# ntampellini/FIRECODE

Measured on AMD Instinct MI355X. Metric: conformer-pair RMSD alignments/s, higher is better.
Workload: dtype f64

## Files before the change

firecode_amd/csrc/fc_api_prune.cpp:

```cpp
#include <algorithm>
#include <chrono>
#include <cmath>
#include <cstdlib>
#include <functional>
#include <memory>

#include "fc_internal.h"
#include "fc_kabsch_math.h"

namespace fc {

struct LadderKs {
  int n;
  int64_t k[24];
};
__global__ void k_store_ladder_ks(LadderKs a, int64_t *__restrict__ out) {
  if ((int)threadIdx.x < a.n) out[threadIdx.x] = a.k[threadIdx.x];
}

static int make_selection(const uint8_t *atom_mask, int64_t A_all, std::vector<int32_t> &sel) {
  sel.clear();
  for (int64_t a = 0; a < A_all; ++a)
    if (atom_mask == nullptr || atom_mask[a]) sel.push_back((int32_t)a);
  if (sel.empty()) return set_error(FC_E_INVALID, "atom_mask selects no atom");
// ... 307 lines not shown
    FC_TRY(sync());
  }
  unpack_ladder_result(e, words, cnt_host, job.mask_out, job.levels, job.survivors, job.counters_out);
  return FC_OK;
}

static void note_candidates(fc_ensemble *e, unsigned long long refined, unsigned long long similar) {
  int guard = 0;
  for (fc_ensemble *w = e->head ? e->head : e; w != nullptr && guard < 8; w = w->twin, ++guard) {
    w->last_candidates = (int64_t)refined;
    w->last_similar = (int64_t)similar;
  }
  Context &c = ctx();
  c.hint_A = e->A, c.hint_N = e->N, c.hint_candidates = (int64_t)refined, c.hint_similar = (int64_t)similar;
}

static bool ladder_collect(fc_ensemble *e, int64_t slot, uint8_t *mask_out, int64_t *levels,
                           int64_t *survivors, unsigned long long *counters_out, int64_t slot_stride = 0) {
  const uint64_t *words = slot_words(slot, e->W, slot_stride), *cnt_host = slot_counters(slot, e->W, slot_stride);
  note_candidates(e, cnt_host[6], cnt_host[2]);
  if (cnt_host[9] == 0) return false;
  unpack_ladder_result(e, words, cnt_host, mask_out, levels, survivors, counters_out);
  return true;
}

static int ensemble_twin(fc_ensemble *ens, fc_ensemble **out) {
  if (!ens->twin) {
    std::unique_ptr<fc_ensemble> t(new (std::nothrow) fc_ensemble);
    if (!t) return set_error(FC_E_NOMEM, "host allocation failed");
    t->epoch = ens->epoch;
    t->N = ens->N, t->A = ens->A, t->Npad = ens->Npad, t->W = ens->W;
    t->Xs.alias(ens->Xs), t->Xa.alias(ens->Xa), t->G.alias(ens->G);
    if (ens->xsf_valid) t->Xsf.alias(ens->Xsf), t->sub.alias(ens->sub), t->xsf_valid = true;
    if (ens->xh_valid) t->Xh.alias(ens->Xh), t->xh_valid = true, t->xh_scale = ens->xh_scale;
    t->g_max = ens->g_max;
    t->head = ens->head ? ens->head : ens;
    t->last_candidates = ens->last_candidates, t->last_similar = ens->last_similar;
    FC_TRY(t->counters.reserve(kCounters * sizeof(uint64_t)));
    ens->twin = t.release();
  }
  *out = ens->twin;
  return FC_OK;
}

static int64_t owned_pairs(int64_t N, int64_t row_block, int64_t rank, int64_t world) {
  int64_t n = 0;
  const int64_t nb = ceil_div(N, row_block);
  for (int64_t lb = 0, b; (b = global_block(lb, rank, world)) < nb; ++lb)
    for (int64_t i = b * row_block; i < std::min(N, (b + 1) * row_block); ++i) n += N - 1 - i;
  return n;
}
static int64_t owned_pairs(const fc_ensemble *ens) { return owned_pairs(ens->N, ens->row_block, ens->rank, ens->world); }

static void fill_stats(int64_t *stats, int64_t pairs, const unsigned long long *cnt, int64_t s4, int64_t s5) {
  stats[0] = pairs, stats[1] = (int64_t)cnt[1], stats[2] = (int64_t)cnt[2], stats[3] = (int64_t)cnt[3];
  stats[4] = s4, stats[5] = s5;
}

static int ladder_workspace(fc_ensemble *e, int64_t N, size_t *bits_bytes = nullptr) {
  e->N = N, e->Npad = ceil_div(N, 64) * 64, e->W = e->Npad / 64;
  e->row_block = 64;
  FC_TRY(e->maskA.reserve((size_t)e->Npad));
  FC_TRY(e->maskB.reserve((size_t)e->Npad));
  FC_TRY(e->mbits.reserve((size_t)e->W * sizeof(uint64_t)));
  FC_TRY(e->counters.reserve(kCounters * sizeof(uint64_t)));
  const int64_t rows = ceil_div(N, e->row_block) * e->row_block;
// ... 1836 lines not shown
```

firecode_amd/csrc/fc_common.h:

```cpp
#pragma once

#include <hip/hip_runtime.h>

#include <cstdarg>
#include <cstdint>
#include <cstdio>
#include <cstring>
#include <mutex>
#include <new>
#include <string>
#include <vector>

#include "../../include/fc_hip.h"
#include "fc_items.h"
#include "fc_tuning.h"

namespace fc {

std::string &last_error();
int set_error(int code, const char *fmt, ...);

#define FC_HIP_TRY(expr)                                                              \
  do {                                                                                \
    hipError_t _e = (expr);                                                           \
// ... 215 lines not shown
  int64_t ref_stride = 0;
  const uint64_t *ref_bits = nullptr;
  const int64_t *excl_offsets = nullptr;
  const int64_t *excl_atoms = nullptr;
  int64_t excl_sets = 0;
  int64_t max_newbonds = 0;
  int64_t *counts_out = nullptr;
  uint8_t *ok_out = nullptr;
  const int64_t *offsets = nullptr;
  int64_t *bonds_out = nullptr;
};
int bond_changes(const BondJob &job);

constexpr double kScreenMargin = 1e-6;
constexpr unsigned long long kRefineLanesMin = 1ull << 17;

constexpr size_t kCounters = 64 + 20 * 16;
constexpr int kCntLevel = 64, kCntLevelStride = 16;


}

struct fc_ensemble {
  uint64_t epoch = 0;
  int64_t N = 0, A = 0;
  int64_t Npad = 0, W = 0;
  fc::DevBuf Xs;
  fc::DevBuf Xa;
  fc::DevBuf G;
  fc::DevBuf Xsf;
  fc::DevBuf sub;
  fc::DevBuf unitq;
  bool xsf_valid = false;
  fc::DevBuf Xh;
  bool xh_valid = false;
  double xh_scale = 0.0;
  double g_max = -1.0;
  bool g_max_pending = false;
  std::vector<int32_t> sel_host;
  fc::DevBuf bits;
  fc::DevBuf cand;
  fc::DevBuf pairq;
  int64_t pairq_cap = 0;
  fc::DevBuf simq;
  fc::DevBuf bk, bk_off, bk_list, sortq;
  int64_t bk_buckets = 0;
  int64_t last_candidates = -1;
  int64_t last_similar = -1;
  fc::DevBuf bits_full;
  fc::DevBuf item_table;
  int64_t item_key[4] = {-1, -1, -1, -1}, item_total = 0;
  std::vector<uint64_t> item_host;
  fc::DevBuf gathered;
  fc::DevBuf msg_send, msg_recv;
  fc::DevBuf energies;
  fc::DevBuf maskA, maskB;
  fc::DevBuf mbits;
  fc::DevBuf ladder;
  fc::DevBuf ladder_k;
  fc::DevBuf levelmask;
  std::vector<int64_t> ladder_k_host;
  int ladder_k_n = -1;
  int64_t ladder_k_mpg = -1;
  fc::DevBuf counters;
  int64_t rank = 0, world = 1, row_block = 64;
  int64_t rows_local = 0;
// ... 11 lines not shown
```

firecode_amd/csrc/fc_items.h:

```cpp
#pragma once

#include <algorithm>
#include <cstdint>
#include <utility>
#include <vector>

#if defined(__HIPCC__) || defined(__CUDACC__)
#define FC_ITEMS_HD __host__ __device__
#else
#define FC_ITEMS_HD
#endif

namespace fc {

FC_ITEMS_HD inline int64_t global_block(int64_t local_block, int64_t rank, int64_t world) {
  return local_block * world + ((local_block & 1) ? (world - 1 - rank) : rank);
}
inline int64_t local_block_count(int64_t n_gblocks, int64_t rank, int64_t world) {
  int64_t n = 0;
  while (global_block(n, rank, world) < n_gblocks) ++n;
  return n;
}

constexpr uint64_t kItemFirstHalf = 1ull << 31, kItemSecondHalf = 1ull << 63;
constexpr int kItemChunkShift = 58, kItemChunkMax = 16;
FC_ITEMS_HD inline int64_t item_tile(uint64_t it) { return (int64_t)(it & 0x7fffffffull); }
FC_ITEMS_HD inline int64_t item_block(uint64_t it) { return (int64_t)((it >> 32) & 0x3ffffffull); }
FC_ITEMS_HD inline int item_blocks(uint64_t it) { return (int)((it >> kItemChunkShift) & 15ull) + 1; }

struct ItemPlan {
  int64_t N = 0, rank = 0, world = 1;
  int64_t row_block = 128, tc = 64;
  int64_t NT = 0, n_lblocks = 0;
  bool halves = false;
  int64_t tail = 0;
  bool real_columns_only = false;
  int64_t chunk = 1;
  bool tail_order = true;
};

template <class F>
inline void item_units(uint64_t it, const ItemPlan &p, F visit) {
  const int64_t jt = item_tile(it), lb = item_block(it), j0 = jt * p.tc, tpb = p.row_block / 16;
  int64_t it_first = 0, it_last = tpb * item_blocks(it);
  if (it & kItemFirstHalf) it_last = tpb / 2;
  if (it & kItemSecondHalf) it_first = tpb / 2;
  const int64_t i0 = global_block(lb, p.rank, p.world) * p.row_block;
  if (i0 >= p.N || j0 + p.tc - 1 <= i0) return;
  for (int64_t t = it_first; t < it_last; ++t) {
    const int64_t ib = global_block(lb + t / tpb, p.rank, p.world) * p.row_block + (t % tpb) * 16;
    if (ib >= p.N) break;
    if (j0 + p.tc - 1 <= ib) break;
    for (int64_t cs = 0; cs < p.tc / 16; ++cs) {
      if (j0 + (cs + 1) * 16 - 1 <= ib) continue;
      if (j0 + cs * 16 >= p.N) continue;
      visit(ib, j0 + cs * 16);
    }
  }
}

inline std::vector<uint64_t> build_items(const ItemPlan &p) {
// ... 46 lines not shown
```

firecode_amd/csrc/fc_kabsch.hip:

```cpp
#include <type_traits>

#include "fc_internal.h"
#include <vector>
#include "fc_kabsch_math.h"

#include <algorithm>
#include <cstdlib>

namespace fc {

__global__ void __launch_bounds__(256)
k_prep(const double *__restrict__ coords, int64_t N, int64_t A_all, const int32_t *__restrict__ sel,
       int64_t A, int center, int64_t Npad, double *__restrict__ Xs, double *__restrict__ G,
       double *__restrict__ Xa, unsigned long long *__restrict__ gmax_bits,
       const int32_t *__restrict__ conf_idx) {
  const int64_t n = (int64_t)blockIdx.x * blockDim.x + threadIdx.x;
  if (n >= Npad) return;
  for (int64_t a = A; a < ((A + 3) & ~(int64_t)3); ++a) {
    Xs[(a * 3 + 0) * Npad + n] = 0.0;
    Xs[(a * 3 + 1) * Npad + n] = 0.0;
    Xs[(a * 3 + 2) * Npad + n] = 0.0;
  }
  if (n >= N) {
    for (int64_t a = 0; a < A; ++a) {
// ... 525 lines not shown
        acc[k][0] = fma(x, qx, acc[k][0]);
        acc[k][1] = fma(x, qy, acc[k][1]);
        acc[k][2] = fma(x, qz, acc[k][2]);
        acc[k][3] = fma(y, qx, acc[k][3]);
        acc[k][4] = fma(y, qy, acc[k][4]);
        acc[k][5] = fma(y, qz, acc[k][5]);
        acc[k][6] = fma(z, qx, acc[k][6]);
        acc[k][7] = fma(z, qy, acc[k][7]);
        acc[k][8] = fma(z, qz, acc[k][8]);
      }
    }
#pragma unroll
    for (int k = 0; k < TI; ++k) {
      const int64_t i = ib + k;
      const double Gp = G[i];
      bool may = kabsch_may_be_below<ENANT>(acc[k], Gp + Gq, A_thr2);
      may = may && (j > i) && (j < N) && (i < N);
      const uint64_t word = __ballot(may);
      push_pairs(word, may, (unsigned)i, (unsigned)j, pairq, Q, counters, lane);
      if (lane == 0 && i < N) {
        const int64_t lrow = (int64_t)(lb * IB) + (int64_t)it * TI + k;
        bits[lrow * W + jt] = word;
        if (word) {
          const unsigned long long slot = atomicAdd(&counters[4], 1ull);
          cand[slot] = (uint32_t)(lrow * W + jt);
        }
      }
    }
  }
}

typedef double d4_t __attribute__((ext_vector_type(4)));

template <int NW, int MODE = 0, int TC = 64, bool EIG = false, bool ENANT = false>
__global__ void __launch_bounds__(NW * 64, 2)
k_simbits_screen_mfma(const double *__restrict__ Xs, const double *__restrict__ G, int64_t N,
                      int64_t Npad, int A, double A_thr2, int IB, int64_t rank, int64_t world,
                      uint64_t *__restrict__ bits, int64_t W, uint32_t *__restrict__ cand,
                      unsigned long long *__restrict__ counters, uint64_t *__restrict__ pairq,
                      unsigned long long Q, const uint64_t *__restrict__ item_table, unsigned long long n_items,
                      double *__restrict__ rmsd_out = nullptr, const unsigned long long *__restrict__ gate = nullptr,
                      double *__restrict__ maxdev_out = nullptr) {
  static_assert(!EIG || MODE == 2, "EIG: the complete alignments");
  static_assert(!ENANT || MODE == 0, "ENANT: the screen only");
  constexpr bool VALUES = MODE != 0;
  constexpr int NT = MODE == 2 ? 1 : 2;
  static_assert(TC == 64 || ((TC == 32 || TC == 16) && MODE == 2), "column tiles: 64, or 32 / 16 for the complete alignments");
  constexpr int NU = (TC / 16) / NT;
  constexpr int KPR = TC == 64 ? 2 : 4;
  constexpr int SST = 2048 / TC;
  constexpr int CST = TC == 64 ? 256 : 128;
  auto koff = [](int sl) { return TC == 16 ? (sl >> 1) * 384 + (sl & 1) * 64 : sl * (12 * TC); };
  if (gate != nullptr && *gate == 0ull) return;
  extern __shared__ double lds[];
  const int tid = threadIdx.x;
  const int lane = tid & 63;
  const int wv = __builtin_amdgcn_readfirstlane(tid >> 6);
  const int KS = (A + 3) >> 2;
  double *__restrict__ ldsG = lds + (TC == 16 ? ((KS + 1) >> 1) * 384 : KS * 12 * TC);
  uint64_t *__restrict__ stageQ = reinterpret_cast<uint64_t *>(ldsG + TC + IB);
  uint32_t *__restrict__ stageW = reinterpret_cast<uint32_t *>(stageQ + kStagePairs);
  unsigned *__restrict__ stageN = reinterpret_cast<unsigned *>(stageW + kStageWords);
#ifdef FC_TIMELINE
  unsigned long long *tl = MODE == 2 ? reinterpret_cast<unsigned long long *>(bits) : reinterpret_cast<unsigned long long *>(rmsd_out);
  constexpr bool TL = MODE == 0 || MODE == 2;
#endif
  const unsigned long long b = blockIdx.x;
  if (b >= n_items) return;
#ifdef FC_TIMELINE
  if (TL && tl && tid == 0) {
    tl[(size_t)b * 4] = wall_clock64();
    tl[(size_t)b * 4 + 3] = b;
  }
#endif
  int64_t jt, lb;
  int it_first = 0, it_last = IB >> 4;
// ... 191 lines not shown
          {
            double B4[4][9], GG[4], Q44[4][4], nq4[4], lam4[4];
#pragma unroll
            for (int r = 0; r < 4; ++r) {
              GG[r] = Gp + ldsG[cs * 16 + 4 * kq + r];
#pragma unroll
              for (int e = 0; e < 9; ++e) B4[r][e] = acc[t][e][r];
            }
            kabsch_quaternion_qcp_lean4(B4, GG, Q44, nq4, ok4, EIG ? lam4 : nullptr);
            if constexpr (EIG) {
              const double k_small = 2e-10 / (double)A;
#pragma unroll
              for (int r = 0; r < 4; ++r) {
                msdA4[r] = GG[r] - 2.0 * lam4[r];
                if (!(msdA4[r] > k_small * GG[r] * GG[r])) ok4[r] = false, msdA4[r] = 0.0;
              }
            }
#pragma unroll
            for (int r = 0; r < 4; ++r) {
              if (!ok4[r]) Q44[r][0] = 1.0, Q44[r][1] = 0.0, Q44[r][2] = 0.0, Q44[r][3] = 0.0, nq4[r] = 1.0;
              neg_rotation_from_raw_quaternion(Q44[r], nq4[r], nR[r]);
            }
          }
          typedef double d2_t __attribute__((ext_vector_type(2)));
          const double *__restrict__ qcol = lds + cs * SST + 4 * kq;
          const double *__restrict__ prow_u = Xs + ib;
          const unsigned l15u = (unsigned)l15;
          const int n_rounds = (A + 1) >> 1, n_groups = n_rounds >> 1;
          const bool odd_round = (n_rounds & 1) != 0;
          double ssq[4] = {0.0, 0.0, 0.0, 0.0}, mx[4] = {0.0, 0.0, 0.0, 0.0};
          const int64_t Npad3 = 3 * Npad;
          const double *__restrict__ pa0 = prow_u, *__restrict__ pa1 = prow_u + Npad, *__restrict__ pa2 = prow_u + 2 * Npad;
          const double *__restrict__ qg = qcol;
          auto load_pq = [&](auto u_, double (&P)[3], d2_t (&Qv)[3][2]) {
            constexpr int u = decltype(u_)::value;
            const double *__restrict__ ql = qg + (u / KPR) * 128 + (u % KPR) * 16;
#pragma unroll
            for (int c = 0; c < 3; ++c) {
              Qv[c][0] = *reinterpret_cast<const d2_t *>(ql + c * CST);
              Qv[c][1] = *reinterpret_cast<const d2_t *>(ql + c * CST + 2);
            }
            P[0] = pa0[l15u];
            P[1] = pa1[l15u];
            P[2] = pa2[l15u];
            pa0 += Npad3;
            pa1 += Npad3;
            pa2 += Npad3;
          };
          auto accumulate = [&](const double (&P)[3], const d2_t (&Qv)[3][2]) {
#pragma clang fp contract(fast)
#pragma unroll
            for (int r = 0; r < 4; ++r) {
              const double qx = Qv[0][r >> 1][r & 1], qy = Qv[1][r >> 1][r & 1], qz = Qv[2][r >> 1][r & 1];
              const double dx = fma(nR[r][0], qx, fma(nR[r][1], qy, fma(nR[r][2], qz, P[0])));
              const double dy = fma(nR[r][3], qx, fma(nR[r][4], qy, fma(nR[r][5], qz, P[1])));
              const double dz = fma(nR[r][6], qx, fma(nR[r][7], qy, fma(nR[r][8], qz, P[2])));
              const double s2 = fma(dz, dz, fma(dy, dy, dx * dx));
              if constexpr (!EIG) ssq[r] += s2;
              asm("v_max_f64 %0, %1, %2" : "=v"(mx[r]) : "v"(mx[r]), "v"(s2));
            }
          };
          using U0 = std::integral_constant<int, 0>;
          using U1 = std::integral_constant<int, 1>;
          using U2 = std::integral_constant<int, 2>;
          using U3 = std::integral_constant<int, 3>;
          double PA[3], PB[3];
          d2_t QA[3][2], QB[3][2];
          load_pq(U0{}, PA, QA);
          for (int g = 0; g < n_groups; ++g) {
            load_pq(U1{}, PB, QB);
            __builtin_amdgcn_sched_barrier(0);
            accumulate(PA, QA);
            __builtin_amdgcn_sched_barrier(0);
            load_pq(U2{}, PA, QA);
            __builtin_amdgcn_sched_barrier(0);
            accumulate(PB, QB);
            __builtin_amdgcn_sched_barrier(0);
            load_pq(U3{}, PB, QB);
            __builtin_amdgcn_sched_barrier(0);
            accumulate(PA, QA);
            __builtin_amdgcn_sched_barrier(0);
            qg = TC == 16 ? qcol + koff(g + 1) : qg + 12 * TC;
            if (g + 1 < n_groups || odd_round) load_pq(U0{}, PA, QA);
            __builtin_amdgcn_sched_barrier(0);
            accumulate(PB, QB);
            __builtin_amdgcn_sched_barrier(0);
          }
          if (odd_round) {
            load_pq(U1{}, PB, QB);
            __builtin_amdgcn_sched_barrier(0);
            accumulate(PA, QA);
            __builtin_amdgcn_sched_barrier(0);
            accumulate(PB, QB);
          }
          if constexpr (EIG) {
#pragma unroll
            for (int r = 0; r < 4; ++r) ssq[r] = msdA4[r];
          }
          const bool row_in = i < n32;
          double *__restrict__ ro = rmsd_out + (int64_t)i * N + jb;
          double *__restrict__ mo = maxdev_out + (int64_t)i * N + jb;
          const double invA = 1.0 / (double)A;
          if (row_in && jb > i && jb + 3 < n32 && ((((int64_t)i * N) & 1) == 0)) {
            *reinterpret_cast<d2_t *>(ro) = d2_t{fc_sqrt_nonneg(ssq[0] * invA), fc_sqrt_nonneg(ssq[1] * invA)};
            *reinterpret_cast<d2_t *>(ro + 2) = d2_t{fc_sqrt_nonneg(ssq[2] * invA), fc_sqrt_nonneg(ssq[3] * invA)};
            *reinterpret_cast<d2_t *>(mo) = d2_t{fc_sqrt_nonneg(mx[0]), fc_sqrt_nonneg(mx[1])};
            *reinterpret_cast<d2_t *>(mo + 2) = d2_t{fc_sqrt_nonneg(mx[2]), fc_sqrt_nonneg(mx[3])};
          } else {
#pragma unroll
            for (int r = 0; r < 4; ++r) {
              const int j = jb + r;
              if (row_in && j >= i && j < n32) {
                ro[r] = j == i ? 0.0 : fc_sqrt_nonneg(ssq[r] * invA);
                mo[r] = j == i ? 0.0 : fc_sqrt_nonneg(mx[r]);
              }
            }
          }
#pragma unroll
          for (int r = 0; r < 4; ++r) {
            const int j = jb + r;
            const bool redo = row_in && (j > i) && (j < n32) && !ok4[r];
            stage_pairs(__ballot(redo), redo, (unsigned)i, (unsigned)j, stageQ, stageN, pairq, Q, counters, lane);
          }
          continue;
        }
#pragma unroll
        for (int r = 0; r < 4; ++r) {
// ... 1751 lines not shown

static int screen_item_table(fc_ensemble *e, int64_t NT, int64_t n_lblocks, bool halves = true, int64_t tc = 64, int64_t chunk = 0,
                             bool tail_order = true) {
  const int64_t rb_key = (((e->row_block * 2 + (halves ? 1 : 0)) * 128 + tc) * 32 + chunk) * 2 + (tail_order ? 1 : 0);
  if (e->item_key[0] == e->N && e->item_key[1] == e->rank && e->item_key[2] == e->world &&
      e->item_key[3] == rb_key)
    return FC_OK;
  e->item_total = 0;
  e->item_key[0] = e->N; e->item_key[1] = e->rank; e->item_key[2] = e->world; e->item_key[3] = rb_key;
  ItemPlan plan;
  plan.N = e->N; plan.rank = e->rank; plan.world = e->world;
  plan.row_block = e->row_block; plan.tc = tc; plan.NT = NT; plan.n_lblocks = n_lblocks;
  plan.tail = 2 * (int64_t)ctx().n_cu;
  if (const char *v = getenv("FC_SCREEN_TAIL_SLOTS")) plan.tail = std::max<int64_t>(0, std::strtoll(v, nullptr, 10));
  plan.halves = halves && e->row_block == 128 && e->A <= 52;
  plan.real_columns_only = chunk > 0;
  plan.chunk = std::max<int64_t>(1, chunk);
  plan.tail_order = tail_order;
  std::vector<uint64_t> items = build_items(plan);
  if (items.empty() || items.size() >= (1ull << 31)) return FC_OK;
  FC_TRY(e->item_table.reserve(items.size() * sizeof(uint64_t)));
  e->item_host.swap(items);
  FC_TRY(h2d(e->item_table.p, e->item_host.data(), e->item_host.size() * sizeof(uint64_t)));
  e->item_total = (int64_t)e->item_host.size();
  return FC_OK;
}

int prebuild_screen_items(fc_ensemble *e) {
  const int64_t n_lblocks = local_block_count(ceil_div(e->N, e->row_block), e->rank, e->world);
  if (n_lblocks <= 0 || (e->Npad >> 6) == 0) return FC_OK;
  return screen_item_table(e, e->Npad >> 6, n_lblocks, true, 64);
}

template <int NW, int TC, bool EIG>
static int launch_complete_variant(fc_ensemble *e, dim3 grid, size_t lds_m, double A_small, int64_t rb, int64_t rank, int64_t world,
                                   unsigned long long *cnt, const uint64_t *item_table_dev, unsigned long long n_items,
                                   double *rmsd_dev, double *maxdev_dev, uint64_t *timeline_dev) {
  if (lds_m > 64 * 1024) {
    hipError_t err = hipFuncSetAttribute(reinterpret_cast<const void *>(k_simbits_screen_mfma<NW, 2, TC, EIG>),
                                         hipFuncAttributeMaxDynamicSharedMemorySize, (int)lds_m);
    if (err != hipSuccess) return set_error(FC_E_HIP, "hipFuncSetAttribute failed: %s", hipGetErrorString(err));
  }
  hipLaunchKernelGGL((k_simbits_screen_mfma<NW, 2, TC, EIG>), grid, dim3(NW * 64), lds_m, ctx().stream, e->Xs.as<double>(),
                     e->G.as<double>(), e->N, e->Npad, (int)e->A, A_small, (int)rb, rank, world, timeline_dev, e->W, nullptr, cnt,
                     e->pairq.as<uint64_t>(), (unsigned long long)e->pairq_cap, item_table_dev, n_items, rmsd_dev, nullptr,
                     maxdev_dev);
  return FC_OK;
}

int launch_rmsd_values(fc_ensemble *e, double small_rmsd, double *rmsd_dev, double *maxdev_dev, int64_t rank,
                       int64_t world, bool explicit_sum) {
  const int64_t rb = 128;
  const int64_t n_lblocks = local_block_count(ceil_div(e->N, rb), rank, world);
  if (n_lblocks <= 0) return FC_OK;
  const size_t lds_64 = ((size_t)((e->A + 3) / 4) * 4 * 3 * 64 + 64 + (size_t)rb) * sizeof(double) + kStageBytes;
  const size_t lds_32 = ((size_t)((e->A + 3) / 4) * 4 * 3 * 32 + 32 + (size_t)rb) * sizeof(double) + kStageBytes;
  const size_t lds_16 = ((size_t)(((e->A + 3) / 4 + 1) / 2) * 384 + 16 + (size_t)rb) * sizeof(double) + kStageBytes;
  const bool narrow = lds_64 > kLdsLimit && maxdev_dev != nullptr;
  const int64_t tc = !narrow ? 64 : (lds_32 <= kLdsLimit ? 32 : 16);
  const size_t lds_m = tc == 64 ? lds_64 : (tc == 32 ? lds_32 : lds_16);
  const int64_t NT = e->Npad / tc;
  if (lds_m > kLdsLimit || NT == 0)
    return set_error(FC_E_LIMIT, "A=%lld atoms exceed the LDS column tile of the value kernel", (long long)e->A);
  const bool fits32 = (uint64_t)((e->A + 3) / 4 * 4) * 3 * (uint64_t)e->Npad < (1ull << 32) &&
                      96 * (uint64_t)e->Npad < (1ull << 32);
  if (!fits32) return set_error(FC_E_LIMIT, "ensemble too large for 32-bit operand offsets");
  auto *cnt = reinterpret_cast<unsigned long long *>(e->counters.p);
  const bool two_blocks = 2 * lds_m <= kLdsLimit;
  const bool complete = maxdev_dev != nullptr;
  const void *fn = two_blocks ? reinterpret_cast<const void *>(k_simbits_screen_mfma<4, 1>)
                              : reinterpret_cast<const void *>(k_simbits_screen_mfma<8, 1>);
  if (!complete && lds_m > 64 * 1024) {
    hipError_t err = hipFuncSetAttribute(fn, hipFuncAttributeMaxDynamicSharedMemorySize, (int)lds_m);
    if (err != hipSuccess) return set_error(FC_E_HIP, "hipFuncSetAttribute failed: %s", hipGetErrorString(err));
  }
  const double A_small = (double)e->A * small_rmsd * small_rmsd;
  const int64_t saved_rank = e->rank, saved_world = e->world, saved_rb = e->row_block;
  e->rank = rank; e->world = world; e->row_block = rb;
  int64_t chunk = 0;
  bool tail_order = true;
  if (complete) {
    chunk = two_blocks && !narrow ? kCompleteRowChunk : 1;
    if (const char *v = getenv("FC_COMPLETE_ROW_CHUNK")) chunk = std::min<int64_t>(kItemChunkMax, std::max<int64_t>(1, std::strtoll(v, nullptr, 10)));
    if (const char *v = getenv("FC_COMPLETE_TAIL_ORDER")) tail_order = atoi(v) != 0;
  }
  const int rc_tbl = screen_item_table(e, NT, n_lblocks, true, tc, chunk, tail_order);
  e->rank = saved_rank; e->world = saved_world; e->row_block = saved_rb;
  e->item_key[3] = -1;
  if (rc_tbl != FC_OK) return rc_tbl;
  const int compact = e->item_total > 0 ? 1 : 0;
  const unsigned long long n_items =
      compact ? (unsigned long long)e->item_total : (unsigned long long)NT * (unsigned long long)n_lblocks;
  const uint64_t *item_table_dev = compact ? e->item_table.as<uint64_t>() : nullptr;
  if (n_items >= (1ull << 31)) return set_error(FC_E_LIMIT, "too many value-kernel items for one launch");
  const dim3 grid((unsigned)n_items);
  uint64_t *timeline_dev = nullptr;
#ifdef FC_TIMELINE
  static DevBuf tlbuf;
  const bool timeline = complete && getenv("FC_TIMELINE_OUT") != nullptr;
  if (timeline) {
    FC_TRY(tlbuf.reserve(n_items * 4 * sizeof(uint64_t)));
    FC_HIP_TRY(hipMemsetAsync(tlbuf.p, 0, n_items * 4 * sizeof(uint64_t), ctx().stream));
    timeline_dev = tlbuf.as<uint64_t>();
  }
#endif
#define FC_LAUNCH_VALUES(NW_, MODE_)                                                                      \
  hipLaunchKernelGGL((k_simbits_screen_mfma<NW_, MODE_>), grid, dim3(NW_ * 64), lds_m, ctx().stream,      \
                     e->Xs.as<double>(), e->G.as<double>(), e->N, e->Npad, (int)e->A, A_small, (int)rb,   \
                     rank, world, nullptr, e->W, nullptr, cnt, e->pairq.as<uint64_t>(),                   \
                     (unsigned long long)e->pairq_cap, item_table_dev, n_items, rmsd_dev, nullptr, maxdev_dev)
  const char *eig_env = getenv("FC_COMPLETE_EIG");
  const bool eig = complete && !(eig_env && atoi(eig_env) == 0) && !explicit_sum;
#define FC_LAUNCH_COMPLETE(NW_, TC_)                                                                                        \
  FC_TRY((eig ? launch_complete_variant<NW_, TC_, true>(e, grid, lds_m, A_small, rb, rank, world, cnt, item_table_dev, n_items, \
                                                       rmsd_dev, maxdev_dev, timeline_dev)                                 \
              : launch_complete_variant<NW_, TC_, false>(e, grid, lds_m, A_small, rb, rank, world, cnt, item_table_dev,     \
                                                        n_items, rmsd_dev, maxdev_dev, timeline_dev)))
  if (narrow && tc == 32) {
    FC_LAUNCH_COMPLETE(8, 32);
  } else if (narrow) {
    FC_LAUNCH_COMPLETE(8, 16);
  } else if (complete) {
    if (two_blocks) FC_LAUNCH_COMPLETE(4, 64);
    else FC_LAUNCH_COMPLETE(8, 64);
  } else {
    if (two_blocks) FC_LAUNCH_VALUES(4, 1);
    else FC_LAUNCH_VALUES(8, 1);
  }
#undef FC_LAUNCH_COMPLETE
#undef FC_LAUNCH_VALUES
  FC_TRY(check_launch("k_simbits_screen_mfma<values>"));
#ifdef FC_TIMELINE
  if (timeline) {
    std::vector<uint64_t> h(n_items * 4);
    FC_HIP_TRY(hipMemcpyAsync(h.data(), tlbuf.p, h.size() * sizeof(uint64_t), hipMemcpyDeviceToHost, ctx().stream));
    FC_HIP_TRY(hipStreamSynchronize(ctx().stream));
    if (FILE *f = fopen(getenv("FC_TIMELINE_OUT"), "wb")) {
      const uint64_t head[2] = {(uint64_t)n_items, compact ? 1ull : 0ull};
      fwrite(head, sizeof(uint64_t), 2, f);
      fwrite(h.data(), sizeof(uint64_t), h.size(), f);
      if (compact) fwrite(e->item_host.data(), sizeof(uint64_t), e->item_host.size(), f);
      fclose(f);
    }
  }
#endif
  if (ctx().mark_after_screen) (void)hipEventRecord(ctx().mark_after_screen, ctx().stream);
  hipLaunchKernelGGL(k_rmsd_fix_small, dim3((unsigned)(ctx().n_cu * 4)), dim3(256), 0, ctx().stream,
                     e->Xa.as<double>(), (int)e->A, e->N, e->pairq.as<uint64_t>(), cnt,
                     (unsigned long long)e->pairq_cap, rmsd_dev, maxdev_dev);
  return check_launch("k_rmsd_fix_small");
}

__global__ void __launch_bounds__(256)
k_gather_matrix_pairs(const double *__restrict__ rmsd_m, const double *__restrict__ maxdev_m, int64_t N,
                      const int64_t *__restrict__ pi, const int64_t *__restrict__ pj, int64_t P,
                      double *__restrict__ rmsd_out, double *__restrict__ maxdev_out) {
  const int64_t p = (int64_t)blockIdx.x * blockDim.x + threadIdx.x;
  if (p >= P) return;
  int64_t i = pi[p], j = pj[p];
  if (i > j) { const int64_t t = i; i = j; j = t; }
  rmsd_out[p] = rmsd_m[i * N + j];
  maxdev_out[p] = maxdev_m[i * N + j];
// ... 13 lines not shown
  const int64_t bi = blockIdx.y, bj = blockIdx.x;
  if (bj < bi) return;
  const int tx = threadIdx.x & 31, ty = threadIdx.x >> 5;
  for (int r = ty; r < 32; r += 8) {
    const int64_t i = bi * 32 + r, j = bj * 32 + tx;
    tile[r][tx] = (i < N && j < N) ? m[i * N + j] : 0.0;
  }
  __syncthreads();
  for (int r = ty; r < 32; r += 8) {
    const int64_t j = bj * 32 + r, i = bi * 32 + tx;
    if (i < N && j < N && j > i) m[j * N + i] = tile[tx][r];
  }
}

int launch_mirror_upper(double *m_dev, int64_t N) {
  if (N < 2) return FC_OK;
  const unsigned nb = (unsigned)ceil_div(N, 32);
  hipLaunchKernelGGL(k_mirror_upper, dim3(nb, nb), dim3(256), 0, ctx().stream, m_dev, N);
  return check_launch("k_mirror_upper");
}

int launch_scatter_pairs(const uint64_t *pairs_dev, int64_t n_pairs, int64_t N, int64_t W,
                         uint64_t *bits_dev) {
  if (n_pairs == 0) return FC_OK;
  hipLaunchKernelGGL(k_scatter_pairs, dim3((unsigned)ceil_div(n_pairs, 256)), dim3(256), 0,
                     ctx().stream, pairs_dev, n_pairs, N, W, bits_dev);
  return check_launch("k_scatter_pairs");
}

int launch_prep_begin(fc_ensemble *e) {
  auto *gmax_bits = reinterpret_cast<unsigned long long *>(e->counters.p) + (kCounters - 1);
  FC_HIP_TRY(hipMemsetAsync(gmax_bits, 0, sizeof(unsigned long long), ctx().stream));
  e->xsf_valid = false;
  e->xh_valid = false;
  e->g_max = -1.0;
  return FC_OK;
}
bool prep_by_tiles(int64_t A_all) {
  const size_t lds_tile = (size_t)kPrepTile * (size_t)(A_all * 3 + 1) * sizeof(double) + (size_t)A_all * sizeof(int) + 8;
  return lds_tile + 2048 <= kLdsLimit && (uint64_t)kPrepTile * (uint64_t)(A_all * 3 + 1) < (1ull << 31) &&
         !getenv("FC_PREP_LANES");
}
int launch_prep_tiles(const double *coords_dev, int64_t N, int64_t A_all, const int32_t *sel_dev, int64_t A, int center,
                      fc_ensemble *e, const int32_t *conf_idx_dev, int64_t tile0, int64_t n_tiles) {
  if (n_tiles <= 0) return FC_OK;
  auto *gmax_bits = reinterpret_cast<unsigned long long *>(e->counters.p) + (kCounters - 1);
  constexpr int64_t kPer64 = 64 / kPrepTile;
  const size_t lds_tile = (size_t)kPrepTile * (size_t)(A_all * 3 + 1) * sizeof(double) + (size_t)A_all * sizeof(int) + 8;
  if (lds_tile > 64 * 1024)
    FC_HIP_TRY(hipFuncSetAttribute(reinterpret_cast<const void *>(k_prep_tile<kPrepTile>),
                                   hipFuncAttributeMaxDynamicSharedMemorySize, (int)lds_tile));
  hipLaunchKernelGGL(k_prep_tile<kPrepTile>, dim3((unsigned)(n_tiles * kPer64)), dim3(256), lds_tile, ctx().stream, coords_dev, N,
                     A_all, sel_dev, A, center, e->Npad, e->Xs.as<double>(), e->G.as<double>(), e->Xa.as<double>(), gmax_bits,
                     conf_idx_dev, tile0 * kPer64);
  return check_launch("k_prep_tile");
}
int launch_prep_body(const double *coords_dev, int64_t N, int64_t A_all, const int32_t *sel_dev, int64_t A, int center,
                     fc_ensemble *e, const int32_t *conf_idx_dev);
int launch_prep(const double *coords_dev, int64_t N, int64_t A_all, const int32_t *sel_dev,
                int64_t A, int center, fc_ensemble *e, const int32_t *conf_idx_dev) {
  FC_TRY(launch_prep_begin(e));
  return launch_prep_body(coords_dev, N, A_all, sel_dev, A, center, e, conf_idx_dev);
}
int launch_prep_body(const double *coords_dev, int64_t N, int64_t A_all, const int32_t *sel_dev, int64_t A, int center,
                     fc_ensemble *e, const int32_t *conf_idx_dev) {
  if (prep_by_tiles(A_all))
// ... 392 lines not shown
  return e->enant ? launch_f32_screen_of<true>(e, p, n_lblocks, A_thr2) : launch_f32_screen_of<false>(e, p, n_lblocks, A_thr2);
}

static int launch_fp64_screen(fc_ensemble *e, const ScreenPlan &p, int64_t n_lblocks, double A_thr2,
                              const unsigned long long *gate) {
  const auto fn = e->enant ? (p.fp64_waves == 4 ? k_simbits_screen_mfma<4, 0, 64, false, true> : k_simbits_screen_mfma<8, 0, 64, false, true>)
                            : (p.fp64_waves == 4 ? k_simbits_screen_mfma<4> : k_simbits_screen_mfma<8>);
  const int threads = 64 * p.fp64_waves;
  if (p.lds64 > 64 * 1024) {
    hipError_t err = hipFuncSetAttribute(reinterpret_cast<const void *>(fn), hipFuncAttributeMaxDynamicSharedMemorySize,
                                         (int)p.lds64);
    if (err != hipSuccess)
      return set_error(FC_E_HIP, "hipFuncSetAttribute(LDS=%zu) failed: %s", p.lds64, hipGetErrorString(err));
  }
  if (getenv("FC_DEBUG")) {
    int nb = -1;
    (void)hipOccupancyMaxActiveBlocksPerMultiprocessor(&nb, reinterpret_cast<const void *>(fn), threads, p.lds64);
    fprintf(stderr, "[fc] screen_mfma<%d>: LDS %zu B, occupancy API says %d blocks/CU\n", p.fp64_waves, p.lds64, nb);
  }
  ScreenItems it;
  FC_TRY(screen_items(e, n_lblocks, 64, &it));
  double *dbg = nullptr;
#ifdef FC_TIMELINE
  static DevBuf tlbuf;
  if (p.timeline) {
    FC_TRY(tlbuf.reserve(it.n * 4 * sizeof(unsigned long long)));
    FC_HIP_TRY(hipMemsetAsync(tlbuf.p, 0, it.n * 4 * sizeof(unsigned long long), ctx().stream));
    dbg = tlbuf.as<double>();
  }
#endif
  hipLaunchKernelGGL(fn, dim3((unsigned)it.n), dim3(threads), p.lds64, ctx().stream, e->Xs.as<double>(), e->G.as<double>(), e->N,
                     e->Npad, (int)e->A, A_thr2, (int)e->row_block, e->rank, e->world, e->bits.as<uint64_t>(), e->W,
                     e->cand.as<uint32_t>(), reinterpret_cast<unsigned long long *>(e->counters.p), e->pairq.as<uint64_t>(),
                     (unsigned long long)e->pairq_cap, it.table, it.n, dbg, gate, nullptr);
  FC_TRY(check_launch("k_simbits_screen_mfma"));
#ifdef FC_TIMELINE
  if (p.timeline) {
    std::vector<unsigned long long> h(it.n * 4);
    FC_HIP_TRY(hipMemcpyAsync(h.data(), tlbuf.p, it.n * 4 * sizeof(unsigned long long), hipMemcpyDeviceToHost, ctx().stream));
    FC_HIP_TRY(hipStreamSynchronize(ctx().stream));
    if (FILE *f = fopen(getenv("FC_TIMELINE_OUT"), "wb")) {
      fwrite(h.data(), sizeof(unsigned long long), h.size(), f);
      fclose(f);
    }
  }
#endif
  return FC_OK;
}

static int launch_valu_screen(fc_ensemble *e, const ScreenPlan &p, int64_t n_lblocks, double A_thr2) {
  const auto fn = e->enant ? (p.valu_lds ? k_simbits_screen<true, 8, 4, true> : k_simbits_screen<false, 8, 4, true>)
                            : (p.valu_lds ? k_simbits_screen<true, 8, 4> : k_simbits_screen<false, 8, 4>);
  if (p.lds > 64 * 1024) {
    hipError_t err = hipFuncSetAttribute(reinterpret_cast<const void *>(fn), hipFuncAttributeMaxDynamicSharedMemorySize, (int)p.lds);
    if (err != hipSuccess)
      return set_error(FC_E_HIP, "hipFuncSetAttribute(LDS=%zu) failed: %s", p.lds, hipGetErrorString(err));
  }
  hipLaunchKernelGGL(fn, dim3((unsigned)(e->Npad >> 6), (unsigned)n_lblocks), dim3(256), p.lds, ctx().stream, e->Xs.as<double>(),
                     e->G.as<double>(), e->N, e->Npad, (int)e->A, A_thr2, (int)e->row_block, e->rank, e->world,
                     e->bits.as<uint64_t>(), e->W, e->cand.as<uint32_t>(), reinterpret_cast<unsigned long long *>(e->counters.p),
                     e->pairq.as<uint64_t>(), (unsigned long long)e->pairq_cap);
  return check_launch("k_simbits_screen");
}

int launch_simbits_screen(fc_ensemble *e, double thr2_margin) {
  auto mark_main = []() {
    if (ctx().mark_after_screen) (void)hipEventRecord(ctx().mark_after_screen, ctx().stream);
// ... 164 lines not shown
```

Measured before the change: 20.45 billion.

## Add row-tiled coordinate copy for complete-alignment residual pass with explicit waitcnt pipelining

Builds a row-tiled, interleaved copy of the selected coordinates (16 conformers by atom pairs by xyz, packed as d2 vectors) once per ensemble. The complete-alignment MFMA kernel then reads the P-side coordinates from it as 16-byte vector loads, replacing three strided scalar loads per atom. The residual loop is rescheduled with explicit s_waitcnt so loads overlap the FMA accumulation. The path is on by default and adds an extra buffer, a one-time transpose kernel, and more template instantiations.

After: 20.99 billion, median of 6. 2.6% higher.

```diff
diff --git a/firecode_amd/csrc/fc_api_prune.cpp b/firecode_amd/csrc/fc_api_prune.cpp
--- a/firecode_amd/csrc/fc_api_prune.cpp
+++ b/firecode_amd/csrc/fc_api_prune.cpp
@@ -363,6 +363,7 @@
     t->N = ens->N, t->A = ens->A, t->Npad = ens->Npad, t->W = ens->W;
     t->Xs.alias(ens->Xs), t->Xa.alias(ens->Xa), t->G.alias(ens->G);
     if (ens->xsf_valid) t->Xsf.alias(ens->Xsf), t->sub.alias(ens->sub), t->xsf_valid = true;
+    if (ens->xt_valid) t->Xt.alias(ens->Xt), t->xt_valid = true;
     if (ens->xh_valid) t->Xh.alias(ens->Xh), t->xh_valid = true, t->xh_scale = ens->xh_scale;
     t->g_max = ens->g_max;
     t->head = ens->head ? ens->head : ens;
diff --git a/firecode_amd/csrc/fc_common.h b/firecode_amd/csrc/fc_common.h
--- a/firecode_amd/csrc/fc_common.h
+++ b/firecode_amd/csrc/fc_common.h
@@ -271,6 +271,8 @@
   fc::DevBuf sub;
   fc::DevBuf unitq;
   bool xsf_valid = false;
+  fc::DevBuf Xt;
+  bool xt_valid = false;
   fc::DevBuf Xh;
   bool xh_valid = false;
   double xh_scale = 0.0;
diff --git a/firecode_amd/csrc/fc_items.h b/firecode_amd/csrc/fc_items.h
--- a/firecode_amd/csrc/fc_items.h
+++ b/firecode_amd/csrc/fc_items.h
@@ -27,6 +27,12 @@
 FC_ITEMS_HD inline int64_t item_tile(uint64_t it) { return (int64_t)(it & 0x7fffffffull); }
 FC_ITEMS_HD inline int64_t item_block(uint64_t it) { return (int64_t)((it >> 32) & 0x3ffffffull); }
 FC_ITEMS_HD inline int item_blocks(uint64_t it) { return (int)((it >> kItemChunkShift) & 15ull) + 1; }
+
+FC_ITEMS_HD inline int64_t row_tile_pairs(int64_t A) { return (A + 1) / 2; }
+FC_ITEMS_HD inline int64_t row_tile_offset(int64_t n, int64_t a, int64_t c, int64_t A) {
+  return (((n >> 4) * row_tile_pairs(A) + (a >> 1)) * 3 + c) * 32 + (n & 15) * 2 + (a & 1);
+}
+FC_ITEMS_HD inline int64_t row_tile_elems(int64_t Npad, int64_t A) { return (Npad >> 4) * row_tile_pairs(A) * 96; }
 
 struct ItemPlan {
   int64_t N = 0, rank = 0, world = 1;
diff --git a/firecode_amd/csrc/fc_kabsch.hip b/firecode_amd/csrc/fc_kabsch.hip
--- a/firecode_amd/csrc/fc_kabsch.hip
+++ b/firecode_amd/csrc/fc_kabsch.hip
@@ -581,7 +581,7 @@
 
 typedef double d4_t __attribute__((ext_vector_type(4)));
 
-template <int NW, int MODE = 0, int TC = 64, bool EIG = false, bool ENANT = false>
+template <int NW, int MODE = 0, int TC = 64, bool EIG = false, bool ENANT = false, bool ROWT = false>
 __global__ void __launch_bounds__(NW * 64, 2)
 k_simbits_screen_mfma(const double *__restrict__ Xs, const double *__restrict__ G, int64_t N,
                       int64_t Npad, int A, double A_thr2, int IB, int64_t rank, int64_t world,
@@ -589,8 +589,9 @@
                       unsigned long long *__restrict__ counters, uint64_t *__restrict__ pairq,
                       unsigned long long Q, const uint64_t *__restrict__ item_table, unsigned long long n_items,
                       double *__restrict__ rmsd_out = nullptr, const unsigned long long *__restrict__ gate = nullptr,
-                      double *__restrict__ maxdev_out = nullptr) {
+                      double *__restrict__ maxdev_out = nullptr, const double *__restrict__ Xt = nullptr) {
   static_assert(!EIG || MODE == 2, "EIG: the complete alignments");
+  static_assert(!ROWT || MODE == 2, "ROWT: the complete alignments");
   static_assert(!ENANT || MODE == 0, "ENANT: the screen only");
   constexpr bool VALUES = MODE != 0;
   constexpr int NT = MODE == 2 ? 1 : 2;
@@ -848,7 +849,7 @@
           const int64_t Npad3 = 3 * Npad;
           const double *__restrict__ pa0 = prow_u, *__restrict__ pa1 = prow_u + Npad, *__restrict__ pa2 = prow_u + 2 * Npad;
           const double *__restrict__ qg = qcol;
-          auto load_pq = [&](auto u_, double (&P)[3], d2_t (&Qv)[3][2]) {
+          auto load_q = [&](auto u_, d2_t (&Qv)[3][2]) {
             constexpr int u = decltype(u_)::value;
             const double *__restrict__ ql = qg + (u / KPR) * 128 + (u % KPR) * 16;
 #pragma unroll
@@ -856,6 +857,9 @@
               Qv[c][0] = *reinterpret_cast<const d2_t *>(ql + c * CST);
               Qv[c][1] = *reinterpret_cast<const d2_t *>(ql + c * CST + 2);
             }
+          };
+          auto load_pq = [&](auto u_, double (&P)[3], d2_t (&Qv)[3][2]) {
+            load_q(u_, Qv);
             P[0] = pa0[l15u];
             P[1] = pa1[l15u];
             P[2] = pa2[l15u];
@@ -863,14 +867,14 @@
             pa1 += Npad3;
             pa2 += Npad3;
           };
-          auto accumulate = [&](const double (&P)[3], const d2_t (&Qv)[3][2]) {
+          auto accumulate3 = [&](const double px, const double py, const double pz, const d2_t (&Qv)[3][2]) {
 #pragma clang fp contract(fast)
 #pragma unroll
             for (int r = 0; r < 4; ++r) {
               const double qx = Qv[0][r >> 1][r & 1], qy = Qv[1][r >> 1][r & 1], qz = Qv[2][r >> 1][r & 1];
-              const double dx = fma(nR[r][0], qx, fma(nR[r][1], qy, fma(nR[r][2], qz, P[0])));
-              const double dy = fma(nR[r][3], qx, fma(nR[r][4], qy, fma(nR[r][5], qz, P[1])));
-              const double dz = fma(nR[r][6], qx, fma(nR[r][7], qy, fma(nR[r][8], qz, P[2])));
+              const double dx = fma(nR[r][0], qx, fma(nR[r][1], qy, fma(nR[r][2], qz, px)));
+              const double dy = fma(nR[r][3], qx, fma(nR[r][4], qy, fma(nR[r][5], qz, py)));
+              const double dz = fma(nR[r][6], qx, fma(nR[r][7], qy, fma(nR[r][8], qz, pz)));
               const double s2 = fma(dz, dz, fma(dy, dy, dx * dx));
               if constexpr (!EIG) ssq[r] += s2;
               asm("v_max_f64 %0, %1, %2" : "=v"(mx[r]) : "v"(mx[r]), "v"(s2));
@@ -880,35 +884,102 @@
           using U1 = std::integral_constant<int, 1>;
           using U2 = std::integral_constant<int, 2>;
           using U3 = std::integral_constant<int, 3>;
-          double PA[3], PB[3];
           d2_t QA[3][2], QB[3][2];
-          load_pq(U0{}, PA, QA);
-          for (int g = 0; g < n_groups; ++g) {
-            load_pq(U1{}, PB, QB);
-            __builtin_amdgcn_sched_barrier(0);
-            accumulate(PA, QA);
-            __builtin_amdgcn_sched_barrier(0);
-            load_pq(U2{}, PA, QA);
-            __builtin_amdgcn_sched_barrier(0);
-            accumulate(PB, QB);
-            __builtin_amdgcn_sched_barrier(0);
-            load_pq(U3{}, PB, QB);
-            __builtin_amdgcn_sched_barrier(0);
-            accumulate(PA, QA);
-            __builtin_amdgcn_sched_barrier(0);
-            qg = TC == 16 ? qcol + koff(g + 1) : qg + 12 * TC;
-            if (g + 1 < n_groups || odd_round) load_pq(U0{}, PA, QA);
-            __builtin_amdgcn_sched_barrier(0);
-            accumulate(PB, QB);
-            __builtin_amdgcn_sched_barrier(0);
+#define FC_SB __builtin_amdgcn_sched_barrier(0)
+          if constexpr (ROWT) {
+            const char *__restrict__ pt = reinterpret_cast<const char *>(Xt) + (ib >> 4) * ((int64_t)n_rounds * 768);
+            unsigned lo = l15u * 16u;
+            auto load_t = [&](auto rho_, d2_t (&T)[3]) {
+              constexpr int rho = decltype(rho_)::value;
+              asm volatile("" : "+v"(lo));
+#pragma unroll
+              for (int c = 0; c < 3; ++c) T[c] = *reinterpret_cast<const d2_t *>(pt + lo + (rho * 768 + c * 256));
+            };
+            auto wait_for = [&](auto vm_, auto lgkm_) {
+              constexpr int vm = decltype(vm_)::value, lgkm = decltype(lgkm_)::value;
+              __builtin_amdgcn_s_waitcnt((vm & 15) | ((vm >> 4) << 14) | (7 << 4) | (lgkm << 8));
+              FC_SB;
+            };
+            auto accumulate = [&](auto h_, const d2_t (&T)[3], const d2_t (&Qv)[3][2]) {
+              constexpr int h = decltype(h_)::value;
+              accumulate3(T[0][h], T[1][h], T[2][h], Qv);
+            };
+            using W0 = std::integral_constant<int, 0>;
+            using W3 = std::integral_constant<int, 3>;
+            using W6 = std::integral_constant<int, 6>;
+            using WX = std::integral_constant<int, 63>;
+            d2_t T0[3], T1[3];
+            const int g_more = odd_round ? n_groups : n_groups - 1;
+            load_q(U0{}, QA);
+            load_t(U0{}, T0);
+            for (int g = 0; g < n_groups; ++g) {
+              load_q(U1{}, QB);
+              load_t(U1{}, T1);
+              FC_SB;
+              wait_for(W3{}, W6{});
+              accumulate(U0{}, T0, QA);
+              FC_SB;
+              load_q(U2{}, QA);
+              FC_SB;
+              wait_for(WX{}, W6{});
+              accumulate(U1{}, T0, QB);
+              FC_SB;
+              load_q(U3{}, QB);
+              pt += 1536;
+              load_t(U0{}, T0);
+              FC_SB;
+              wait_for(W3{}, W6{});
+              accumulate(U0{}, T1, QA);
+              FC_SB;
+              const int gn = g < g_more ? g + 1 : g;
+              qg = TC == 16 ? qcol + koff(gn) : qg + (gn - g) * (12 * TC);
+              load_q(U0{}, QA);
+              FC_SB;
+              wait_for(WX{}, W6{});
+              accumulate(U1{}, T1, QB);
+              FC_SB;
+            }
+            if (odd_round) {
+              load_q(U1{}, QB);
+              FC_SB;
+              wait_for(W0{}, W6{});
+              accumulate(U0{}, T0, QA);
+              FC_SB;
+              wait_for(WX{}, W0{});
+              accumulate(U1{}, T0, QB);
+            }
+          } else {
+            auto accumulate = [&](const double (&P)[3], const d2_t (&Qv)[3][2]) { accumulate3(P[0], P[1], P[2], Qv); };
+            double PA[3], PB[3];
+            load_pq(U0{}, PA, QA);
+            for (int g = 0; g < n_groups; ++g) {
+              load_pq(U1{}, PB, QB);
+              FC_SB;
+              accumulate(PA, QA);
+              FC_SB;
+              load_pq(U2{}, PA, QA);
+              FC_SB;
+              accumulate(PB, QB);
+              FC_SB;
+              load_pq(U3{}, PB, QB);
+              FC_SB;
+              accumulate(PA, QA);
+              FC_SB;
+              qg = TC == 16 ? qcol + koff(g + 1) : qg + 12 * TC;
+              if (g + 1 < n_groups || odd_round) load_pq(U0{}, PA, QA);
+              FC_SB;
+              accumulate(PB, QB);
+              FC_SB;
+            }
+            if (odd_round) {
+              load_pq(U1{}, PB, QB);
+              FC_SB;
+              accumulate(PA, QA);
+              FC_SB;
+              accumulate(PB, QB);
+            }
           }
-          if (odd_round) {
-            load_pq(U1{}, PB, QB);
-            __builtin_amdgcn_sched_barrier(0);
-            accumulate(PA, QA);
-            __builtin_amdgcn_sched_barrier(0);
-            accumulate(PB, QB);
-          }
+#undef FC_SB
           if constexpr (EIG) {
 #pragma unroll
             for (int r = 0; r < 4; ++r) ssq[r] = msdA4[r];
@@ -2726,19 +2797,50 @@
   return screen_item_table(e, e->Npad >> 6, n_lblocks, true, 64);
 }
 
-template <int NW, int TC, bool EIG>
+__global__ void __launch_bounds__(256)
+k_row_tiles(const double *__restrict__ Xs, int64_t Npad, int A, int64_t n_elems, int64_t n_alloc, double *__restrict__ Xt) {
+  const int64_t idx = (int64_t)blockIdx.x * blockDim.x + threadIdx.x;
+  if (idx >= n_alloc) return;
+  double v = 0.0;
+  if (idx < n_elems) {
+    const int64_t U = row_tile_pairs(A), q = idx >> 5, tu = q / 3;
+    const int64_t c = q - tu * 3, t = tu / U, u = tu - t * U;
+    const int64_t n = t * 16 + ((idx >> 1) & 15), a = 2 * u + (idx & 1);
+    if (a < A) v = Xs[(a * 3 + c) * Npad + n];
+  }
+  Xt[idx] = v;
+}
+
+static bool row_tiles_fit(int64_t Npad, int64_t A) {
+  const int64_t n_alloc = row_tile_elems(Npad, A) + 96;
+  return row_tile_pairs(A) * 768 < ((int64_t)1 << 31) && grid_x_fits(ceil_div(n_alloc, 256), 256);
+}
+static int make_row_tiles(fc_ensemble *e) {
+  if (e->xt_valid) return FC_OK;
+  if (!row_tiles_fit(e->Npad, e->A)) return set_error(FC_E_LIMIT, "ensemble too large for the row-tile copy");
+  const int64_t n_elems = row_tile_elems(e->Npad, e->A), n_alloc = n_elems + 96;
+  FC_TRY(e->Xt.reserve((size_t)n_alloc * sizeof(double)));
+  hipLaunchKernelGGL(k_row_tiles, dim3((unsigned)ceil_div(n_alloc, 256)), dim3(256), 0, ctx().stream, e->Xs.as<double>(), e->Npad,
+                     (int)e->A, n_elems, n_alloc, e->Xt.as<double>());
+  FC_TRY(check_launch("k_row_tiles"));
+  e->xt_valid = true;
+  return FC_OK;
+}
+
+template <int NW, int TC, bool EIG, bool ROWT>
 static int launch_complete_variant(fc_ensemble *e, dim3 grid, size_t lds_m, double A_small, int64_t rb, int64_t rank, int64_t world,
                                    unsigned long long *cnt, const uint64_t *item_table_dev, unsigned long long n_items,
                                    double *rmsd_dev, double *maxdev_dev, uint64_t *timeline_dev) {
   if (lds_m > 64 * 1024) {
-    hipError_t err = hipFuncSetAttribute(reinterpret_cast<const void *>(k_simbits_screen_mfma<NW, 2, TC, EIG>),
+    hipError_t err = hipFuncSetAttribute(reinterpret_cast<const void *>(k_simbits_screen_mfma<NW, 2, TC, EIG, false, ROWT>),
                                          hipFuncAttributeMaxDynamicSharedMemorySize, (int)lds_m);
     if (err != hipSuccess) return set_error(FC_E_HIP, "hipFuncSetAttribute failed: %s", hipGetErrorString(err));
   }
-  hipLaunchKernelGGL((k_simbits_screen_mfma<NW, 2, TC, EIG>), grid, dim3(NW * 64), lds_m, ctx().stream, e->Xs.as<double>(),
+  hipLaunchKernelGGL((k_simbits_screen_mfma<NW, 2, TC, EIG, false, ROWT>), grid, dim3(NW * 64), lds_m, ctx().stream, e->Xs.as<double>(),
                      e->G.as<double>(), e->N, e->Npad, (int)e->A, A_small, (int)rb, rank, world, timeline_dev, e->W, nullptr, cnt,
                      e->pairq.as<uint64_t>(), (unsigned long long)e->pairq_cap, item_table_dev, n_items, rmsd_dev, nullptr,
-                     maxdev_dev);
+                     maxdev_dev,
+                     ROWT ? e->Xt.as<double>() : nullptr);
   return FC_OK;
 }
 
@@ -2805,11 +2907,15 @@
                      (unsigned long long)e->pairq_cap, item_table_dev, n_items, rmsd_dev, nullptr, maxdev_dev)
   const char *eig_env = getenv("FC_COMPLETE_EIG");
   const bool eig = complete && !(eig_env && atoi(eig_env) == 0) && !explicit_sum;
+  const char *rt_env = getenv("FC_COMPLETE_ROW_TILES");
+  const bool row_tiles = complete && !(rt_env && atoi(rt_env) == 0);
+  if (row_tiles) FC_TRY(make_row_tiles(e));
+#define FC_COMPLETE_ARGS e, grid, lds_m, A_small, rb, rank, world, cnt, item_table_dev, n_items, rmsd_dev, maxdev_dev, timeline_dev
 #define FC_LAUNCH_COMPLETE(NW_, TC_)                                                                                        \
-  FC_TRY((eig ? launch_complete_variant<NW_, TC_, true>(e, grid, lds_m, A_small, rb, rank, world, cnt, item_table_dev, n_items, \
-                                                       rmsd_dev, maxdev_dev, timeline_dev)                                 \
-              : launch_complete_variant<NW_, TC_, false>(e, grid, lds_m, A_small, rb, rank, world, cnt, item_table_dev,     \
-                                                        n_items, rmsd_dev, maxdev_dev, timeline_dev)))
+  FC_TRY((eig ? (row_tiles ? launch_complete_variant<NW_, TC_, true, true>(FC_COMPLETE_ARGS)                                  \
+                           : launch_complete_variant<NW_, TC_, true, false>(FC_COMPLETE_ARGS))                                \
+              : (row_tiles ? launch_complete_variant<NW_, TC_, false, true>(FC_COMPLETE_ARGS)                                 \
+                           : launch_complete_variant<NW_, TC_, false, false>(FC_COMPLETE_ARGS))))
   if (narrow && tc == 32) {
     FC_LAUNCH_COMPLETE(8, 32);
   } else if (narrow) {
@@ -2822,6 +2928,7 @@
     else FC_LAUNCH_VALUES(8, 1);
   }
 #undef FC_LAUNCH_COMPLETE
+#undef FC_COMPLETE_ARGS
 #undef FC_LAUNCH_VALUES
   FC_TRY(check_launch("k_simbits_screen_mfma<values>"));
 #ifdef FC_TIMELINE
@@ -2901,6 +3008,7 @@
   auto *gmax_bits = reinterpret_cast<unsigned long long *>(e->counters.p) + (kCounters - 1);
   FC_HIP_TRY(hipMemsetAsync(gmax_bits, 0, sizeof(unsigned long long), ctx().stream));
   e->xsf_valid = false;
+  e->xt_valid = false;
   e->xh_valid = false;
   e->g_max = -1.0;
   return FC_OK;
@@ -3359,7 +3467,7 @@
   hipLaunchKernelGGL(fn, dim3((unsigned)it.n), dim3(threads), p.lds64, ctx().stream, e->Xs.as<double>(), e->G.as<double>(), e->N,
                      e->Npad, (int)e->A, A_thr2, (int)e->row_block, e->rank, e->world, e->bits.as<uint64_t>(), e->W,
                      e->cand.as<uint32_t>(), reinterpret_cast<unsigned long long *>(e->counters.p), e->pairq.as<uint64_t>(),
-                     (unsigned long long)e->pairq_cap, it.table, it.n, dbg, gate, nullptr);
+                     (unsigned long long)e->pairq_cap, it.table, it.n, dbg, gate, nullptr, nullptr);
   FC_TRY(check_launch("k_simbits_screen_mfma"));
 #ifdef FC_TIMELINE
   if (p.timeline) {
```
